# wondmgezahu/RAMP

Hardware: AMD Instinct MI355X
Metric: sampled trajectories/sec (H=48, T=25) (higher is better)
Workload: dtype f32-emulated (2 x fp16 planes per operand, fp32 accumulate)

## Files before the change

### ramp_amd/build.py

```python
from __future__ import annotations

import os
import re
import subprocess
import sys
from concurrent.futures import ThreadPoolExecutor

HERE = os.path.dirname(os.path.abspath(__file__))
CSRC = os.path.join(HERE, "csrc")
LIBDIR = os.path.join(HERE, "lib")
LIB = os.path.join(LIBDIR, "libramp_hip.so")
TOOLS_LIB = os.path.join(LIBDIR, "libramp_hip_tools.so")
SOURCES = ["gemm.hip", "ffx.hip", "ffx16.hip", "tkl.hip", "tkl16.hip", "atk.hip", "atb.hip", "atl.hip", "tkc.hip", "tkw.hip", "rowops.hip", "attention.hip", "sampler.hip", "guide.hip", "guide_replan.hip", "guide_prims.hip", "stitch.hip", "resample.hip", "clearance.hip", "scene.hip", "metrics.hip", "engine.hip", "ops.hip"]
TOOLS_SOURCES = ["bench.hip"]
FLAGS = ["--offload-arch=gfx950", "-O3", "-std=c++17", "-fPIC", "-Wno-unused-result", "-DRAMP_DEFAULT_GEMM_MODE=2"]
EXTRA_FLAGS = {"sampler.hip": ["-ffp-contract=off"], "guide.hip": ["-ffp-contract=off"], "guide_replan.hip": ["-ffp-contract=off"], "guide_prims.hip": ["-ffp-contract=off"], "resample.hip": ["-ffp-contract=off"], "clearance.hip": ["-ffp-contract=off"], "stitch.hip": ["-ffp-contract=off"], "ffx.hip": ["-fno-slp-vectorize"], "ffx16.hip": ["-fno-slp-vectorize"], "tkl.hip": ["-fno-slp-vectorize"], "tkl16.hip": ["-fno-slp-vectorize"], "atk.hip": ["-fno-slp-vectorize", "-mllvm", "-amdgpu-mfma-vgpr-form"], "atb.hip": ["-fno-slp-vectorize"], "atl.hip": ["-fno-slp-vectorize", "-mllvm", "-amdgpu-mfma-vgpr-form"], "tkc.hip": ["-fno-slp-vectorize"], "tkw.hip": ["-fno-slp-vectorize"]}


def _stale(out: str, deps) -> bool:
    if not os.path.exists(out):
        return True
    t = os.path.getmtime(out)
    return any(os.path.getmtime(d) > t for d in deps)


def header_deps():
    import glob
    hs = sorted(glob.glob(os.path.join(CSRC, "*.h")) + glob.glob(os.path.join(CSRC, "*.inc")))
    return hs + [os.path.join(HERE, "..", "include", "ramp_hip.h"), os.path.join(HERE, "..", "include", "ramp_hip_tools.h"), os.path.abspath(__file__)]


_INCLUDE = re.compile(r'^\s*#\s*include\s+"([^"]+)"', re.M)


def source_deps(path: str):
    seen, todo = [], [os.path.normpath(path)]
    while todo:
        f = todo.pop()
        if f in seen or not os.path.exists(f):
            continue
        seen.append(f)
        with open(f, encoding="utf-8") as fh:
            for inc in _INCLUDE.findall(fh.read()):
                todo.append(os.path.normpath(os.path.join(os.path.dirname(f), inc)))
    return seen + [os.path.abspath(__file__)]


def stale_sources(force: bool = False):
    objdir = os.path.join(LIBDIR, "obj")
    jobs = []
    for src in SOURCES + TOOLS_SOURCES:
        sp = os.path.join(CSRC, src)
        op = os.path.join(objdir, src.replace(".hip", ".o"))
        if force or _stale(op, source_deps(sp)):
            jobs.append((sp, op))
    return jobs


def build(force: bool = False, verbose: bool = True) -> str:
    hipcc = os.environ.get("HIPCC", "/opt/rocm/bin/hipcc")
    os.makedirs(LIBDIR, exist_ok=True)
    objdir = os.path.join(LIBDIR, "obj")
    os.makedirs(objdir, exist_ok=True)
    jobs = stale_sources(force)

    def compile_one(job):
        sp, op = job
        cmd = [hipcc] + FLAGS + EXTRA_FLAGS.get(os.path.basename(sp), []) + ["-c", sp, "-o", op]
        r = subprocess.run(cmd, capture_output=True, text=True)
        if r.returncode != 0:
            raise RuntimeError(f"hipcc failed for {sp}:\n{r.stderr[-4000:]}")
        return sp

    if jobs:
        with ThreadPoolExecutor(max_workers=4) as ex:
            for sp in ex.map(compile_one, jobs):
                if verbose:
                    print(f"[ramp_amd.build] compiled {os.path.basename(sp)}", file=sys.stderr)
    objs = [os.path.join(objdir, s.replace(".hip", ".o")) for s in SOURCES]
    tobjs = objs + [os.path.join(objdir, s.replace(".hip", ".o")) for s in TOOLS_SOURCES]
    for lib, oo in ((LIB, objs), (TOOLS_LIB, tobjs)):
        if force or jobs or _stale(lib, oo):
            cmd = [hipcc, "--offload-arch=gfx950", "-shared", "-fPIC", "-o", lib] + oo
            r = subprocess.run(cmd, capture_output=True, text=True)
            if r.returncode != 0:
                raise RuntimeError(f"link failed:\n{r.stderr[-4000:]}")
            if verbose:
                print(f"[ramp_amd.build] linked {lib}", file=sys.stderr)
    return LIB


if __name__ == "__main__":
    build(force="--force" in sys.argv)
```

### ramp_amd/csrc/args_gemm.h

```cpp
#pragma once
#include "core.h"
#include "pack.h"

namespace ramp {

struct GemmArgs {
  const float* A = nullptr;  int lda = 0;
  const float* A2 = nullptr; int lda2 = 0; int K1 = 0;
  const float* W = nullptr;
  const unsigned short* Wx = nullptr; long wx_plane = 0;
  const float* a_absmax_in = nullptr; float* a_absmax_out = nullptr; int* range_flag = nullptr; float w_scale_inv = 1.f;
  int site_id = 0;
  int geglu_group = 64;
  const float* Amul = nullptr; int lda_mul = 0; int a_period = 0;
  int ablate = 0;
  int three_ok = 1;
  int tile_pref = 0;
  int wx_packed = 0;
  const float* bias = nullptr;
  const float* rowbias = nullptr; const int* rowvar = nullptr; int row0 = 0; int rb_stride = 0;
  const float* resid = nullptr;  int ldr = 0;
  const float* resid2 = nullptr; int ldr2 = 0;
  float* C = nullptr;  int ldc = 0;
  float* C2 = nullptr; int ldc2 = 0; int N1 = 0;
  int M = 0, N = 0, K = 0;
  int taps = 1, shift0 = 0, shift_step = 0, L = 1;
  int a_stride = 1, c_rstride = 1, c_roff = 0;
  int epi = 0;
  const float* aux_in = nullptr;
  float* aux_out = nullptr;
  int ld_aux = 0;
};
enum { EPI_LINEAR = 0, EPI_GEGLU_FWD = 1, EPI_GEGLU_BWD = 2 };
int launch_gemm(const GemmArgs& a, hipStream_t s);
int launch_ff_fwd(const GemmArgs& ff1, const GemmArgs& ff2, hipStream_t s);
int init_gemm_attributes();
}
```

### ramp_amd/csrc/gemm.hip

```cpp
#include "args_gemm.h"

#include <algorithm>

namespace ramp {

typedef float f32x16 __attribute__((ext_vector_type(16)));
typedef float f32x4 __attribute__((ext_vector_type(4)));

constexpr int BK = 32;
constexpr int LDS_LD = BK + 4;

__device__ __forceinline__ float gelu_f(float x) { return 0.5f * x * (1.f + erff(x * 0.70710678118654752440f)); }
__device__ __forceinline__ float gelu_grad_f(float x) {
  const float cdf = 0.5f * (1.f + erff(x * 0.70710678118654752440f));
  const float pdf = expf(-0.5f * x * x) * 0.39894228040143267794f;
  return cdf + x * pdf;
}

__device__ __forceinline__ void normal_cdf_pdf(float x, float& cdf, float& pdf) {
  const float ax = fabsf(x);
  const float t = __builtin_amdgcn_rcpf(fmaf(0.2316419f, ax, 1.f));
  pdf = __builtin_amdgcn_exp2f(x * x * -0.72134752044448170368f) * 0.39894228040143267794f;
  float poly = fmaf(1.330274429f, t, -1.821255978f);
  poly = fmaf(poly, t, 1.781477937f);
// ... 926 lines not shown
          }
        }
        parity ^= 1;
      }
      load_w(bw[1], wnext, 0, 1);
      if (a.ablate & 2) {
#pragma unroll
        for (int qq = 0; qq < 4; ++qq) asm volatile("" :: "v"(acc[qq >> 1][qq & 1]));
#pragma unroll
        for (int ni = 0; ni < NI; ++ni) wblk[ni] = wnext[ni];
        __syncthreads();
        continue;
      }
      {
        float* Rw = RAW + wn * (FF_RAW / 4);
#pragma unroll
        for (int mi = 0; mi < MI; ++mi)
#pragma unroll
          for (int ni = 0; ni < NI; ++ni)
#pragma unroll
            for (int reg = 0; reg < 16; ++reg)
              Rw[(mi * 32 + (reg & 3) + 8 * (reg >> 2) + 4 * h) * 68 + ni * 32 + r] = acc[mi][ni][reg];
      }
#pragma unroll
      for (int ni = 0; ni < NI; ++ni) wblk[ni] = wnext[ni];
      __syncthreads();
    }
  } else {
    u32x4 fa[NP][MI], fb[2][NP][NI];
    load_w2(fb[0], 0);
    __syncthreads();
#pragma unroll 1
    for (int it = 0; it < 9; ++it) __syncthreads();
    f32x16 acc[MI][NI];
    for (int cq = 0; cq < Q; ++cq) {
      if ((cq & 7) == 0) {
#pragma unroll
        for (int mi = 0; mi < MI; ++mi)
#pragma unroll
          for (int ni = 0; ni < NI; ++ni)
#pragma unroll
            for (int e = 0; e < 16; ++e) acc[mi][ni][e] = 0.f;
      }
      if (a.ablate & 1) {
#pragma unroll 1
        for (int it = 0; it < 9; ++it) __syncthreads();
        continue;
      }
      const int mtq = mt_begin + (cq >> 3) * mt_step, cidx = cq & 7;
      {
        const float* Rw = RAW + wn * (FF_RAW / 4);
        const int rl0 = lane >> 3, c = (lane & 7) * 4;
        const int nbase = cidx * 256 + wn * 64;
        const int half = a.N >> 1, j0 = cidx * 128 + wn * 32 + c;
        f32x4 ba = {0, 0, 0, 0}, bg = {0, 0, 0, 0};
        if (a.bias) { ba = *reinterpret_cast<const f32x4*>(a.bias + nbase + c); bg = *reinterpret_cast<const f32x4*>(a.bias + nbase + 32 + c); }
        unsigned short* PHw = PH + wn * BUF;
#pragma unroll 1
        for (int it = 0; it < 4; ++it) {
          if (a.ablate & 8) { __syncthreads(); continue; }
#pragma unroll
          for (int p = 0; p < 2; ++p) {
            const int rl = (it * 2 + p) * 8 + rl0, m = mtq * 64 + rl;
            f32x4 av4 = *reinterpret_cast<const f32x4*>(Rw + rl * 68 + c);
            f32x4 gv = *reinterpret_cast<const f32x4*>(Rw + rl * 68 + 32 + c);
            av4 = av4 * oscale1 + ba; gv = gv * oscale1 + bg;
            f32x4 hv, s1, s2;
#pragma unroll
            for (int e = 0; e < 4; ++e) {
              float cdf, pdf;
              normal_cdf_pdf(gv[e], cdf, pdf);
              s1[e] = gv[e] * cdf;
              s2[e] = av4[e] * (cdf + gv[e] * pdf);
              hv[e] = av4[e] * s1[e];
            }
            if (m < a.M) {
              *reinterpret_cast<f32x4*>(a.C + (long)m * a.ldc + j0) = s1;
              *reinterpret_cast<f32x4*>(a.C + (long)m * a.ldc + half + j0) = s2;
            } else {
              hv = f32x4{0, 0, 0, 0};
            }
            amax_h = fmaxf(fmaxf(fabsf(hv[0]), fabsf(hv[1])), amax_h); amax_h = fmaxf(fmaxf(fabsf(hv[2]), fabsf(hv[3])), amax_h);
            scale4(hv, s_h);
            const int c8 = lane & 7;
            const int off = rl * XLD + ((((c8 >> 1) ^ (rl >> 2)) & 3) << 3) + (c8 & 1) * 4;
#pragma unroll
            for (int pp = 0; pp < NP; ++pp) *reinterpret_cast<u32x2*>(PHw + pp * PLANE + off) = peel4<NP>(hv, pp + 1 < NP);
          }
          __syncthreads();
        }
      }
#pragma unroll 1
      for (int it = 0; it < 4; ++it) {
        if (a.ablate & 4) { __syncthreads(); continue; }
        const int kb = cidx * 8 + 2 * it;
        load_w2(fb[1], (kb + 1) & 63);
        read_a(fa, PH + it * BUF, 0);
#pragma unroll
        for (int t3 = 0; t3 < 3; ++t3)
#pragma unroll
          for (int mi = 0; mi < MI; ++mi)
#pragma unroll
            for (int ni = 0; ni < NI; ++ni)
              acc[mi][ni] = mfma_planes<NP>(fa[PA[t3]][mi], fb[0][PB[t3]][ni], acc[mi][ni]);
        load_w2(fb[0], (kb + 2) & 63);
        read_a(fa, PH + it * BUF, 1);
#pragma unroll
        for (int t3 = 0; t3 < 3; ++t3)
#pragma unroll
          for (int mi = 0; mi < MI; ++mi)
#pragma unroll
            for (int ni = 0; ni < NI; ++ni)
              acc[mi][ni] = mfma_planes<NP>(fa[PA[t3]][mi], fb[1][PB[t3]][ni], acc[mi][ni]);
        __syncthreads();
      }
      if ((cq & 7) == 7) {
        epilogue_wave_aux<EPI_LINEAR, false, true, 64, 256, 1>(b, acc, Sw, mtq, 1, lane, 0, wn, r, h, oscale2);
      }
      __syncthreads();
    }
  }

  {
    float mx = G1 ? amax : amax_h;
#pragma unroll
    for (int o = 32; o > 0; o >>= 1) mx = fmaxf(mx, __shfl_xor(mx, o));
    if (lane == 0) {
      const GemmArgs& g = G1 ? a : b;
      const float sc = G1 ? s_a : s_h;
      record_amax(g.a_absmax_out, mx);
      if (g.range_flag && (!(mx * sc < 60000.f) || (mx > 0.f && mx * sc < 0.125f))) atomicMax(g.range_flag, g.site_id + 1);
    }
  }
}

int launch_ff_fwd(const GemmArgs& g1, const GemmArgs& g2, hipStream_t s) {
  auto al16 = [](const void* p) { return (reinterpret_cast<uintptr_t>(p) & 15) == 0; };
  RAMP_REQUIRE(g1.wx_packed == 2 && g2.wx_packed == 2 && g1.Wx && g2.Wx, "fused feed-forward needs the fp16 weight planes");
  RAMP_REQUIRE(g1.K == 256 && g1.N == 2048 && g2.K == 1024 && g2.N == 256 && g1.M == g2.M && g1.M > 0, "fused feed-forward: 256 -> 2 x 1024 -> 256 only");
  RAMP_REQUIRE(g1.geglu_group == 32 && g1.taps == 1 && g2.taps == 1 && !g1.A2 && !g1.Amul && !g2.rowbias && !g2.resid2 && !g2.C2, "fused feed-forward: unsupported operand");
  RAMP_REQUIRE(g1.lda % 4 == 0 && g1.ldc % 4 == 0 && g2.ldc % 4 == 0 && (g2.resid == nullptr || g2.ldr % 4 == 0), "leading dimensions must be multiples of 4 floats");
  RAMP_REQUIRE(al16(g1.A) && al16(g1.Wx) && al16(g2.Wx) && al16(g1.C) && al16(g2.C) && al16(g1.bias) && al16(g2.bias) && al16(g2.resid), "operands must be 16-byte aligned");
  FfFwdArgs f; f.g1 = g1; f.g2 = g2;
  f.g2.N1 = f.g2.N; f.g2.K1 = f.g2.K; f.g1.N1 = f.g1.N; f.g1.K1 = f.g1.K;
  const int n_mtiles = (g1.M + 63) / 64;
  const int nb = std::min(((n_mtiles + 7) / 8) * 8, 256);
  hipLaunchKernelGGL(ff_fwd_kernel, dim3(nb), dim3(512), FF_LDS, s, f, n_mtiles);
  RAMP_HIP_CHECK(hipGetLastError());
  return 0;
}

template <int NP>
__global__ void pack_planes_kernel(const float* __restrict__ W, unsigned short* __restrict__ out, long rows, int K, float scale) {
  const int k8n = K / 8;
  const long total = rows * k8n;
  for (long i = (long)blockIdx.x * 256 + threadIdx.x; i < total; i += (long)gridDim.x * 256) {
    const long row = i / k8n;
    const int k8 = (int)(i - row * k8n);
    f32x4 lo = *reinterpret_cast<const f32x4*>(W + row * K + k8 * 8) * scale;
    f32x4 hi = *reinterpret_cast<const f32x4*>(W + row * K + k8 * 8 + 4) * scale;
    const long blk = (row >> 5) * (K / 16) + (k8 >> 1);
    unsigned short* q = out + blk * (NP * 512) + (((k8 & 1) * 32 + (int)(row & 31)) << 3);
#pragma unroll
    for (int p = 0; p < NP; ++p) {
      const bool sub = p + 1 < NP;
      const u32x2 qa = peel4<NP>(lo, sub), qb = peel4<NP>(hi, sub);
      *reinterpret_cast<u32x4*>(q + p * 512) = u32x4{qa[0], qa[1], qb[0], qb[1]};
    }
  }
}
int launch_pack_x6(const float* W, unsigned short* out, long rows, int K, hipStream_t s) {
  RAMP_REQUIRE(rows > 0 && rows % 32 == 0 && K > 0 && K % 16 == 0, "pack_x6 needs rows % 32 == 0 and K % 16 == 0");
  const long total = rows * (K / 8);
  hipLaunchKernelGGL(pack_planes_kernel<3>, dim3((int)std::min<long>((total + 255) / 256, 8192)), dim3(256), 0, s, W, out, rows, K, 1.f);
  RAMP_HIP_CHECK(hipGetLastError());
  return 0;
}
int launch_pack_h3(const float* W, unsigned short* out, long rows, int K, float scale, hipStream_t s) {
  RAMP_REQUIRE(rows > 0 && rows % 32 == 0 && K > 0 && K % 16 == 0, "pack_h3 needs rows % 32 == 0 and K % 16 == 0");
  const long total = rows * (K / 8);
  hipLaunchKernelGGL(pack_planes_kernel<2>, dim3((int)std::min<long>((total + 255) / 256, 8192)), dim3(256), 0, s, W, out, rows, K, scale);
  RAMP_HIP_CHECK(hipGetLastError());
  return 0;
}

constexpr size_t X6_LDS = std::max<size_t>(6 * (size_t)128 * XLD * 2, (size_t)128 * 132 * 4);
constexpr size_t X6P_LDS3 = 2 * (9216 + 3 * (size_t)128 * XLD * 2);
constexpr size_t X6P_LDS2 = 2 * (9728 + 2 * (size_t)128 * XLD * 2);
constexpr size_t X6P_LDS2R = 2 * (17408 + 2 * (size_t)128 * XLD * 2);
constexpr size_t X6P_LDS2W = 2 * (17408 + 2 * (size_t)64 * XLD * 2);
static_assert(X6P_LDS3 <= X6_LDS, "bf16x6 pipelined layout");

template <int EPI, bool GEN>
static int launch_x6(const GemmArgs& a, hipStream_t s) {
  const bool wide = !GEN && a.wx_packed == 2 && a.N % 256 == 0 && a.tile_pref != 1;
  const int BMt = wide ? 64 : 128, BNt = wide ? 256 : 128;
  const int tiles_m = (a.M + BMt - 1) / BMt, tiles_n = (a.N + BNt - 1) / BNt;
  const int n_tiles = tiles_m * tiles_n;
  const bool three_auto = a.three_ok != 0;
  const bool plain = three_auto && EPI == EPI_LINEAR && wide && !a.Amul && !a.resid && !a.rowbias;
  const bool three = a.wx_packed == 2 && (!a.Amul || wide) &&
                     (EPI == EPI_GEGLU_FWD || a.tile_pref == 3 ||
                      (a.tile_pref == 0 && ((plain && n_tiles >= 3072) || (three_auto && wide && a.Amul && n_tiles > 512 && n_tiles <= 768))));
  const int slots = three ? 768 : 512;
  const int rounds = (n_tiles + slots - 1) / slots;
  const int nb = std::min((((n_tiles + rounds - 1) / rounds + 7) / 8) * 8, slots);
#define X6P_LAUNCH(...) hipLaunchKernelGGL((gemm_x6p_kernel<__VA_ARGS__>), dim3(nb), dim3(256), X6P_LDS3, s, a, tiles_n, n_tiles)
  const bool rec = a.a_absmax_out != nullptr;
  if (a.ablate && a.wx_packed == 2) {
    if constexpr (!GEN && EPI == EPI_LINEAR) {
      const size_t lds = wide ? X6P_LDS2W : X6P_LDS2R;
#define ABL_CASE(V) case V: if (wide) hipLaunchKernelGGL((gemm_x6p_abl_kernel<V, true>), dim3(nb), dim3(256), lds, s, a, tiles_n, n_tiles); \
                            else hipLaunchKernelGGL((gemm_x6p_abl_kernel<V, false>), dim3(nb), dim3(256), lds, s, a, tiles_n, n_tiles); break;
      switch (a.ablate) { ABL_CASE(1) ABL_CASE(2) ABL_CASE(3) ABL_CASE(4) ABL_CASE(7) ABL_CASE(8) ABL_CASE(15) ABL_CASE(16) ABL_CASE(32) ABL_CASE(64) ABL_CASE(128) ABL_CASE(136) ABL_CASE(129) ABL_CASE(130) ABL_CASE(131) ABL_CASE(160) ABL_CASE(192) ABL_CASE(144) ABL_CASE(288) ABL_CASE(416) default: RAMP_REQUIRE(false, "ablation variant not built"); }
#undef ABL_CASE
    }
  } else if (wide) {
    if constexpr (!GEN) {
      if (a.Amul) {
        RAMP_REQUIRE(EPI == EPI_LINEAR && a.a_period > 0 && a.a_period % 32 == 0 && a.K == 2 * a.a_period && a.lda_mul % 4 == 0, "bad A-multiplier operand (K = 2 x period)");
        if constexpr (EPI == EPI_LINEAR) {
          if (three) hipLaunchKernelGGL((gemm_x6p3_kernel<EPI_LINEAR, false, true, 2, true, true, true>), dim3(nb), dim3(256), X6P_LDS2W, s, a, tiles_n, n_tiles);
          else hipLaunchKernelGGL((gemm_x6p_kernel<EPI_LINEAR, false, true, 2, true, true>), dim3(nb), dim3(256), X6P_LDS2W, s, a, tiles_n, n_tiles);
        }
      } else if (three && EPI == EPI_LINEAR && !a.resid && !a.rowbias) hipLaunchKernelGGL((gemm_x6p3_kernel<EPI, false, false, 2, true, true, true>), dim3(nb), dim3(256), X6P_LDS2W, s, a, tiles_n, n_tiles);
      else if (three) hipLaunchKernelGGL((gemm_x6p3_kernel<EPI, false, false, 2, true, true>), dim3(nb), dim3(256), X6P_LDS2W, s, a, tiles_n, n_tiles);
      else hipLaunchKernelGGL((gemm_x6p_kernel<EPI, false, false, 2, true, true>), dim3(nb), dim3(256), X6P_LDS2W, s, a, tiles_n, n_tiles);
    }
  } else if (a.wx_packed && a.Amul) {
    RAMP_REQUIRE(EPI == EPI_LINEAR && !GEN && a.a_period > 0 && a.a_period % 32 == 0 && a.K == 2 * a.a_period && a.lda_mul % 4 == 0, "bad A-multiplier operand (K = 2 x period)");
    if (a.wx_packed == 2) hipLaunchKernelGGL((gemm_x6p_kernel<EPI_LINEAR, false, true, 2, true>), dim3(nb), dim3(256), X6P_LDS2R, s, a, tiles_n, n_tiles);
    else if (rec) X6P_LAUNCH(EPI_LINEAR, false, true, 3, true);
    else X6P_LAUNCH(EPI_LINEAR, false, true, 3, false);
  } else if (three) hipLaunchKernelGGL((gemm_x6p3_kernel<EPI, GEN>), dim3(nb), dim3(256), X6P_LDS2, s, a, tiles_n, n_tiles);
  else if (a.wx_packed == 2) hipLaunchKernelGGL((gemm_x6p_kernel<EPI, GEN, false, 2, true>), dim3(nb), dim3(256), X6P_LDS2R, s, a, tiles_n, n_tiles);
  else if (a.wx_packed && rec) X6P_LAUNCH(EPI, GEN, false, 3, true);
  else if (a.wx_packed) X6P_LAUNCH(EPI, GEN, false, 3, false);
  else hipLaunchKernelGGL((gemm_x6_kernel<EPI, GEN>), dim3(nb), dim3(256), X6_LDS, s, a, tiles_n, n_tiles);
  RAMP_HIP_CHECK(hipGetLastError());
  return 0;
}
template <int EPI, bool GEN>
static int set_attr_x6() {
  RAMP_HIP_CHECK(hipFuncSetAttribute(reinterpret_cast<const void*>(&gemm_x6_kernel<EPI, GEN>),
                                     hipFuncAttributeMaxDynamicSharedMemorySize, (int)X6_LDS));
#define X6P_ATTR(...) RAMP_HIP_CHECK(hipFuncSetAttribute(reinterpret_cast<const void*>(&gemm_x6p_kernel<__VA_ARGS__>), \
                                                         hipFuncAttributeMaxDynamicSharedMemorySize, (int)X6P_LDS3))
  X6P_ATTR(EPI, GEN, false, 3, false);
  X6P_ATTR(EPI, GEN, false, 3, true);
  RAMP_HIP_CHECK(hipFuncSetAttribute(reinterpret_cast<const void*>(&gemm_x6p3_kernel<EPI, GEN>),
                                     hipFuncAttributeMaxDynamicSharedMemorySize, (int)X6P_LDS2));
  RAMP_HIP_CHECK(hipFuncSetAttribute(reinterpret_cast<const void*>(&gemm_x6p_kernel<EPI, GEN, false, 2, true>),
                                     hipFuncAttributeMaxDynamicSharedMemorySize, (int)X6P_LDS2R));
  if constexpr (!GEN) {
    RAMP_HIP_CHECK(hipFuncSetAttribute(reinterpret_cast<const void*>(&gemm_x6p_kernel<EPI, false, false, 2, true, true>),
                                       hipFuncAttributeMaxDynamicSharedMemorySize, (int)X6P_LDS2W));
    RAMP_HIP_CHECK(hipFuncSetAttribute(reinterpret_cast<const void*>(&gemm_x6p3_kernel<EPI, false, false, 2, true, true>),
                                       hipFuncAttributeMaxDynamicSharedMemorySize, (int)X6P_LDS2W));
  }
  return 0;
}
template <int WM, int WN, int MI, int NI> struct Cfg {
  static constexpr int BM = WM * MI * 32, BN = WN * NI * 32;
  static constexpr size_t lds = 2 * (size_t)(BM + BN) * LDS_LD * sizeof(float);
};

template <int WM, int WN, int MI, int NI, int EPI, bool GEN>
static int launch_cfg(const GemmArgs& a, int blocks_per_cu, hipStream_t s) {
  using C = Cfg<WM, WN, MI, NI>;
  const int tiles_m = (a.M + C::BM - 1) / C::BM, tiles_n = (a.N + C::BN - 1) / C::BN;
  const int n_tiles = tiles_m * tiles_n;
  const int slots = 256 * blocks_per_cu;
  const int rounds = (n_tiles + slots - 1) / slots;
  const int nb = std::min((((n_tiles + rounds - 1) / rounds + 7) / 8) * 8, slots);
  hipLaunchKernelGGL((gemm_kernel<WM, WN, MI, NI, EPI, GEN>), dim3(nb), dim3(WM * WN * 64), C::lds, s, a, tiles_n, n_tiles);
  RAMP_HIP_CHECK(hipGetLastError());
  return 0;
}

template <int WM, int WN, int MI, int NI, int EPI, bool GEN>
static int set_attr() {
  RAMP_HIP_CHECK(hipFuncSetAttribute(reinterpret_cast<const void*>(&gemm_kernel<WM, WN, MI, NI, EPI, GEN>),
                                     hipFuncAttributeMaxDynamicSharedMemorySize, (int)Cfg<WM, WN, MI, NI>::lds));
  return 0;
}
int init_gemm_attributes() {
  RAMP_HIP_CHECK(hipFuncSetAttribute(reinterpret_cast<const void*>(&ff_fwd_kernel), hipFuncAttributeMaxDynamicSharedMemorySize, (int)FF_LDS));
  if (int e = set_attr<2, 2, 2, 2, EPI_LINEAR, false>()) return e;
  if (int e = set_attr<2, 2, 2, 2, EPI_LINEAR, true>()) return e;
  if (int e = set_attr<2, 2, 2, 2, EPI_GEGLU_FWD, false>()) return e;
  if (int e = set_attr<2, 2, 2, 2, EPI_GEGLU_BWD, false>()) return e;
  if (int e = set_attr<2, 2, 2, 1, EPI_LINEAR, true>()) return e;
  if (int e = set_attr<4, 1, 1, 1, EPI_LINEAR, true>()) return e;
  X6P_ATTR(EPI_LINEAR, false, true, 3, false);
  X6P_ATTR(EPI_LINEAR, false, true, 3, true);
  RAMP_HIP_CHECK(hipFuncSetAttribute(reinterpret_cast<const void*>(&gemm_x6p_kernel<EPI_LINEAR, false, true, 2, true>),
                                     hipFuncAttributeMaxDynamicSharedMemorySize, (int)X6P_LDS2R));
  RAMP_HIP_CHECK(hipFuncSetAttribute(reinterpret_cast<const void*>(&gemm_x6p_kernel<EPI_LINEAR, false, true, 2, true, true>),
                                     hipFuncAttributeMaxDynamicSharedMemorySize, (int)X6P_LDS2W));
#define ABL_ATTR(V) RAMP_HIP_CHECK(hipFuncSetAttribute(reinterpret_cast<const void*>(&gemm_x6p_abl_kernel<V, true>), hipFuncAttributeMaxDynamicSharedMemorySize, (int)X6P_LDS2W)); \
                    RAMP_HIP_CHECK(hipFuncSetAttribute(reinterpret_cast<const void*>(&gemm_x6p_abl_kernel<V, false>), hipFuncAttributeMaxDynamicSharedMemorySize, (int)X6P_LDS2R));
  ABL_ATTR(1) ABL_ATTR(2) ABL_ATTR(3) ABL_ATTR(4) ABL_ATTR(7) ABL_ATTR(8) ABL_ATTR(15) ABL_ATTR(16) ABL_ATTR(32) ABL_ATTR(64)
#undef ABL_ATTR
  if (int e = set_attr_x6<EPI_LINEAR, false>()) return e;
  if (int e = set_attr_x6<EPI_LINEAR, true>()) return e;
  if (int e = set_attr_x6<EPI_GEGLU_FWD, false>()) return e;
  return set_attr_x6<EPI_GEGLU_BWD, false>();
}

__global__ __launch_bounds__(256) void gemm_narrow_kernel(GemmArgs a) {
  const int n4 = a.N >> 2;
  const long idx = (long)blockIdx.x * 256 + threadIdx.x;
  if (idx >= (long)a.M * n4) return;
  const int m = (int)(idx / n4), n = (int)(idx - (long)m * n4) * 4;
  const int seg = m / a.L, l = m - seg * a.L;
  const int Lin = a.L * a.a_stride;
  f32x4 acc = {0, 0, 0, 0};
  for (int tap = 0; tap < a.taps; ++tap) {
    const int ls = l * a.a_stride + a.shift0 + tap * a.shift_step;
    if (ls < 0 || ls >= Lin) continue;
    const long src = (long)seg * Lin + ls;
    const float* w = a.W + ((long)tap * a.N + n) * a.K;
    for (int k = 0; k < a.K; ++k) {
      const float x = k < a.K1 ? a.A[src * a.lda + k] : a.A2[src * a.lda2 + (k - a.K1)];
#pragma unroll
      for (int j = 0; j < 4; ++j) acc[j] += x * w[(long)j * a.K + k];
    }
  }
  const long orow = (long)m * a.c_rstride + a.c_roff;
  if (a.bias) acc += *reinterpret_cast<const f32x4*>(a.bias + n);
  if (a.rowbias) acc += *reinterpret_cast<const f32x4*>(a.rowbias + (long)a.rowvar[a.row0 + m / a.L] * a.rb_stride + n);
  if (a.resid) acc += *reinterpret_cast<const f32x4*>(a.resid + orow * a.ldr + n);
  if (a.resid2) acc += *reinterpret_cast<const f32x4*>(a.resid2 + orow * a.ldr2 + n);
  if (n < a.N1) *reinterpret_cast<f32x4*>(a.C + orow * a.ldc + n) = acc;
  else *reinterpret_cast<f32x4*>(a.C2 + orow * a.ldc2 + (n - a.N1)) = acc;
}

int launch_gemm(const GemmArgs& a_in, hipStream_t s) {
  GemmArgs a = a_in;
  if (a.A2 == nullptr) a.K1 = a.K;
  if (a.C2 == nullptr) a.N1 = a.N;
  if (a.rb_stride == 0) a.rb_stride = a.N;
  auto al16 = [](const void* p) { return (reinterpret_cast<uintptr_t>(p) & 15) == 0; };
  RAMP_REQUIRE(a.M > 0 && a.N > 0 && a.K > 0 && a.taps >= 1 && a.L >= 1, "bad GEMM dims");
  if (a.K % BK != 0) {
    RAMP_REQUIRE(a.K % 16 == 0 && a.N % 4 == 0 && a.N1 % 4 == 0 && a.epi == EPI_LINEAR && !a.Amul && a.a_stride >= 1 && a.c_rstride >= 1 &&
                 (a.A2 == nullptr || a.K1 > 0) && (a.C2 == nullptr || a.N1 > 0),
                 "narrow GEMM (K % 32 != 0): K a multiple of 16, N and N1 multiples of 4, linear epilogue only");
    RAMP_REQUIRE(al16(a.C) && al16(a.C2) && al16(a.resid) && al16(a.resid2) && al16(a.bias) && al16(a.rowbias) &&
                 a.ldc % 4 == 0 && a.ldc2 % 4 == 0 && a.ldr % 4 == 0 && a.ldr2 % 4 == 0 && a.rb_stride % 4 == 0 &&
                 (a.rowbias == nullptr || a.rowvar != nullptr), "narrow GEMM: outputs and epilogue operands must be 16-byte aligned");
    const long n_out = (long)a.M * (a.N / 4);
    hipLaunchKernelGGL(gemm_narrow_kernel, dim3((unsigned)((n_out + 255) / 256)), dim3(256), 0, s, a);
    RAMP_HIP_CHECK(hipGetLastError());
    return 0;
  }
  RAMP_REQUIRE(a.K % BK == 0 && a.lda % 4 == 0 && a.N % 4 == 0 && a.N1 % 4 == 0,
               "K must be a multiple of 32, N, N1 and lda multiples of 4 floats");
  RAMP_REQUIRE(a.A2 == nullptr || (a.lda2 % 4 == 0 && a.K1 % BK == 0), "split-K source must start on a K tile");
  RAMP_REQUIRE(al16(a.A) && al16(a.W) && al16(a.A2) && al16(a.C) && al16(a.C2) && al16(a.resid) && al16(a.resid2) &&
               al16(a.bias) && al16(a.rowbias) && al16(a.aux_in) && al16(a.aux_out), "GEMM operands must be 16-byte aligned");
  RAMP_REQUIRE(a.ldc % 4 == 0 && a.ldc2 % 4 == 0 && a.ldr % 4 == 0 && a.ldr2 % 4 == 0 && a.ld_aux % 4 == 0 &&
               a.rb_stride % 4 == 0, "leading dimensions must be multiples of 4 floats");
  RAMP_REQUIRE(a.rowbias == nullptr || a.rowvar != nullptr, "rowbias needs rowvar");
  RAMP_REQUIRE(a.a_stride >= 1 && a.c_rstride >= 1, "bad strides");
  const bool gen = a.taps > 1 || a.a_stride != 1 || a.c_rstride != 1 || a.c_roff != 0 || a.A2 || a.C2 || a.resid2 ||
                   a.shift0 != 0;
  const bool x6 = a.Wx != nullptr && (a.N >= 128 || (a.wx_packed && a.N >= 64));
  RAMP_REQUIRE(a.Amul == nullptr || (x6 && a.wx_packed && !gen && a.epi == EPI_LINEAR && al16(a.Amul)),
               "the A-multiplier operand needs the pipelined bf16x6 kernel");
  RAMP_REQUIRE(!x6 || (al16(a.Wx) && a.K % 8 == 0 && (a.wx_packed ? a.N % 32 == 0 : a.wx_plane > 0)), "bad bf16x6 weight planes");
  if (a.epi == EPI_GEGLU_FWD) {
    RAMP_REQUIRE(!gen && a.N % 256 == 0 && a.aux_out && !a.resid && !a.rowbias,
                 "GEGLU-forward epilogue needs a plain linear with N % 256 == 0 and aux_out");
    RAMP_REQUIRE((x6 && a.wx_packed != 0) == (a.geglu_group == 32), "GEGLU weight tiling: [32 a | 32 g] for the pipelined kernels, [64 a | 64 g] otherwise");
    if (x6) return launch_x6<EPI_GEGLU_FWD, false>(a, s);
    return launch_cfg<2, 2, 2, 2, EPI_GEGLU_FWD, false>(a, 2, s);
  }
  if (a.epi == EPI_GEGLU_BWD) {
    RAMP_REQUIRE(!gen && a.N >= 128 && a.aux_in && !a.resid && !a.rowbias && !a.bias,
                 "GEGLU-backward epilogue needs a plain linear with aux_in");
    if (x6) return launch_x6<EPI_GEGLU_BWD, false>(a, s);
    return launch_cfg<2, 2, 2, 2, EPI_GEGLU_BWD, false>(a, 2, s);
  }
  if (x6) return gen ? launch_x6<EPI_LINEAR, true>(a, s) : launch_x6<EPI_LINEAR, false>(a, s);
  if (a.N >= 128) {
    if (!gen) return launch_cfg<2, 2, 2, 2, EPI_LINEAR, false>(a, 2, s);
    return launch_cfg<2, 2, 2, 2, EPI_LINEAR, true>(a, 2, s);
  }
  if (a.N >= 64) return launch_cfg<2, 2, 2, 1, EPI_LINEAR, true>(a, 2, s);
  return launch_cfg<4, 1, 1, 1, EPI_LINEAR, true>(a, 3, s);
}

}
```

Before: 4097.

## Add persistent weight-resident GEMM kernel for large-M narrow linear layers

Adds a persistent kernel that loads the entire packed weight matrix into LDS once per block, then loops over 32-token row groups. Each group's activations are prefetched into registers, and the split-precision MFMA products are computed with a fused bias/scale/residual epilogue. It is routed for plain linear GEMMs with K,N in {64,128,256} and M at or above a threshold. The aim is to avoid re-reading weights per tile and to cut tile-launch overhead for tall, skinny GEMMs. In exchange it uses one wave per EU with large LDS, and an env switch can disable it.

Result: no change. 4109, median of 6 (+0.3%).

```diff
diff --git a/ramp_amd/build.py b/ramp_amd/build.py
--- a/ramp_amd/build.py
+++ b/ramp_amd/build.py
@@ -11,10 +11,10 @@
 LIBDIR = os.path.join(HERE, "lib")
 LIB = os.path.join(LIBDIR, "libramp_hip.so")
 TOOLS_LIB = os.path.join(LIBDIR, "libramp_hip_tools.so")
-SOURCES = ["gemm.hip", "ffx.hip", "ffx16.hip", "tkl.hip", "tkl16.hip", "atk.hip", "atb.hip", "atl.hip", "tkc.hip", "tkw.hip", "rowops.hip", "attention.hip", "sampler.hip", "guide.hip", "guide_replan.hip", "guide_prims.hip", "stitch.hip", "resample.hip", "clearance.hip", "scene.hip", "metrics.hip", "engine.hip", "ops.hip"]
+SOURCES = ["gemm.hip", "gemm_edge.hip", "ffx.hip", "ffx16.hip", "tkl.hip", "tkl16.hip", "atk.hip", "atb.hip", "atl.hip", "tkc.hip", "tkw.hip", "rowops.hip", "attention.hip", "sampler.hip", "guide.hip", "guide_replan.hip", "guide_prims.hip", "stitch.hip", "resample.hip", "clearance.hip", "scene.hip", "metrics.hip", "engine.hip", "ops.hip"]
 TOOLS_SOURCES = ["bench.hip"]
 FLAGS = ["--offload-arch=gfx950", "-O3", "-std=c++17", "-fPIC", "-Wno-unused-result", "-DRAMP_DEFAULT_GEMM_MODE=2"]
-EXTRA_FLAGS = {"sampler.hip": ["-ffp-contract=off"], "guide.hip": ["-ffp-contract=off"], "guide_replan.hip": ["-ffp-contract=off"], "guide_prims.hip": ["-ffp-contract=off"], "resample.hip": ["-ffp-contract=off"], "clearance.hip": ["-ffp-contract=off"], "stitch.hip": ["-ffp-contract=off"], "ffx.hip": ["-fno-slp-vectorize"], "ffx16.hip": ["-fno-slp-vectorize"], "tkl.hip": ["-fno-slp-vectorize"], "tkl16.hip": ["-fno-slp-vectorize"], "atk.hip": ["-fno-slp-vectorize", "-mllvm", "-amdgpu-mfma-vgpr-form"], "atb.hip": ["-fno-slp-vectorize"], "atl.hip": ["-fno-slp-vectorize", "-mllvm", "-amdgpu-mfma-vgpr-form"], "tkc.hip": ["-fno-slp-vectorize"], "tkw.hip": ["-fno-slp-vectorize"]}
+EXTRA_FLAGS = {"sampler.hip": ["-ffp-contract=off"], "guide.hip": ["-ffp-contract=off"], "guide_replan.hip": ["-ffp-contract=off"], "guide_prims.hip": ["-ffp-contract=off"], "resample.hip": ["-ffp-contract=off"], "clearance.hip": ["-ffp-contract=off"], "stitch.hip": ["-ffp-contract=off"], "ffx.hip": ["-fno-slp-vectorize"], "ffx16.hip": ["-fno-slp-vectorize"], "tkl.hip": ["-fno-slp-vectorize"], "tkl16.hip": ["-fno-slp-vectorize"], "gemm_edge.hip": ["-fno-slp-vectorize"], "atk.hip": ["-fno-slp-vectorize", "-mllvm", "-amdgpu-mfma-vgpr-form"], "atb.hip": ["-fno-slp-vectorize"], "atl.hip": ["-fno-slp-vectorize", "-mllvm", "-amdgpu-mfma-vgpr-form"], "tkc.hip": ["-fno-slp-vectorize"], "tkw.hip": ["-fno-slp-vectorize"]}
 
 
 def _stale(out: str, deps) -> bool:
diff --git a/ramp_amd/csrc/args_gemm.h b/ramp_amd/csrc/args_gemm.h
--- a/ramp_amd/csrc/args_gemm.h
+++ b/ramp_amd/csrc/args_gemm.h
@@ -35,4 +35,7 @@
 int launch_gemm(const GemmArgs& a, hipStream_t s);
 int launch_ff_fwd(const GemmArgs& ff1, const GemmArgs& ff2, hipStream_t s);
 int init_gemm_attributes();
+bool gemm_edge_serves(const GemmArgs& a);
+int launch_gemm_edge(const GemmArgs& a, hipStream_t s);
+int init_gemm_edge_attributes();
 }
diff --git a/ramp_amd/csrc/gemm.hip b/ramp_amd/csrc/gemm.hip
--- a/ramp_amd/csrc/gemm.hip
+++ b/ramp_amd/csrc/gemm.hip
@@ -1252,6 +1252,7 @@
                     RAMP_HIP_CHECK(hipFuncSetAttribute(reinterpret_cast<const void*>(&gemm_x6p_abl_kernel<V, false>), hipFuncAttributeMaxDynamicSharedMemorySize, (int)X6P_LDS2R));
   ABL_ATTR(1) ABL_ATTR(2) ABL_ATTR(3) ABL_ATTR(4) ABL_ATTR(7) ABL_ATTR(8) ABL_ATTR(15) ABL_ATTR(16) ABL_ATTR(32) ABL_ATTR(64)
 #undef ABL_ATTR
+  if (int e = init_gemm_edge_attributes()) return e;
   if (int e = set_attr_x6<EPI_LINEAR, false>()) return e;
   if (int e = set_attr_x6<EPI_LINEAR, true>()) return e;
   if (int e = set_attr_x6<EPI_GEGLU_FWD, false>()) return e;
@@ -1333,6 +1334,7 @@
     if (x6) return launch_x6<EPI_GEGLU_BWD, false>(a, s);
     return launch_cfg<2, 2, 2, 2, EPI_GEGLU_BWD, false>(a, 2, s);
   }
+  if (x6 && !gen && gemm_edge_serves(a)) return launch_gemm_edge(a, s);
   if (x6) return gen ? launch_x6<EPI_LINEAR, true>(a, s) : launch_x6<EPI_LINEAR, false>(a, s);
   if (a.N >= 128) {
     if (!gen) return launch_cfg<2, 2, 2, 2, EPI_LINEAR, false>(a, 2, s);
diff --git a/ramp_amd/csrc/gemm_edge.hip b/ramp_amd/csrc/gemm_edge.hip
--- /dev/null
+++ b/ramp_amd/csrc/gemm_edge.hip
@@ -0,0 +1,187 @@
+#include "args_gemm.h"
+#include "tokmma.h"
+
+#include <algorithm>
+#include <cstdlib>
+#include <type_traits>
+
+namespace ramp {
+
+namespace {
+constexpr int GE_TROW = 36;
+constexpr int GE_SCR = 32 * GE_TROW * 4;
+constexpr size_t ge_lds(int K, int N) { return (size_t)K * N * 4 + 4 * GE_SCR + (size_t)N * 4; }
+static_assert(ge_lds(256, 128) <= 160 * 1024 && ge_lds(128, 256) <= 160 * 1024, "LDS budget");
+}
+
+namespace {
+template <int I, int E, class Fn>
+__device__ __forceinline__ void static_for(Fn&& f) {
+  if constexpr (I < E) { f(std::integral_constant<int, I>{}); static_for<I + 1, E>(f); }
+}
+}
+
+template <int K, int N, bool RES>
+__global__ __launch_bounds__(256) __attribute__((amdgpu_waves_per_eu(1, 1)))
+void gemm_edge_kernel(GemmArgs a, int n_groups) {
+  constexpr int NKS = K / 16, NB = N / 32;
+  constexpr int NLD = K / 8;
+  constexpr int W_BYTES = K * N * 4;
+  extern __shared__ __attribute__((aligned(16))) char smem[];
+  const int tid = threadIdx.x, lane = tid & 63;
+  const int wave = __builtin_amdgcn_readfirstlane(tid >> 6);
+  const int t = lane & 31, h = lane >> 5;
+
+  const float s_a = scale_of(a.a_absmax_in);
+  const float os = a.w_scale_inv / s_a;
+  float amax = 0.f;
+
+  f32x4 xn[NLD];
+  auto x_row = [&](int g) __attribute__((always_inline)) {
+    long tok = (long)g * 32 + t;
+    tok = tok < a.M ? tok : a.M - 1;
+    return a.A + tok * a.lda + 8 * h;
+  };
+  const int stride = (int)gridDim.x * 4;
+  int g = (int)blockIdx.x * 4 + wave;
+  {
+    const float* xr = x_row(g);
+#pragma unroll
+    for (int u = 0; u < NLD; ++u) xn[u] = *reinterpret_cast<const f32x4*>(xr + 16 * (u >> 1) + 4 * (u & 1));
+  }
+  {
+    const char* wsrc = reinterpret_cast<const char*>(a.Wx) + lane * 16;
+    const unsigned wdst = (unsigned)(uintptr_t)smem;
+#pragma unroll
+    for (int i = 0; i < W_BYTES / 4096; ++i) {
+      const int piece = 4 * i + wave;
+      asm volatile("s_mov_b32 m0, %1\n\ts_nop 0\n\tglobal_load_lds_dwordx4 %0, off" :: "v"(wsrc + piece * 1024), "s"(wdst + piece * 1024) : "memory", "m0");
+    }
+    float* bsw = reinterpret_cast<float*>(smem + W_BYTES + 4 * GE_SCR);
+    for (int i = tid; i < N; i += 256) bsw[i] = a.bias ? a.bias[i] : 0.f;
+  }
+  asm volatile("s_waitcnt vmcnt(0)" ::: "memory");
+  __syncthreads();
+
+  const char* wrd = smem + lane * 16;
+  const int l8 = lane >> 3, c4 = 4 * (lane & 7);
+  float* tw = reinterpret_cast<float*>(smem + W_BYTES + wave * GE_SCR);
+  float* tw_w = tw + t * GE_TROW + 4 * h;
+  const float* tw_r = tw + l8 * GE_TROW + c4;
+  const float* bs = reinterpret_cast<const float*>(smem + W_BYTES + 4 * GE_SCR) + c4;
+
+  for (; g < n_groups; g += stride) {
+    const float* xr_next = x_row(g + stride < n_groups ? g + stride : g);
+    u32x4 XB[NKS][2];
+#pragma unroll
+    for (int ks = 0; ks < NKS; ++ks) {
+      amax_pin(amax, xn[2 * ks][0], xn[2 * ks][1]); amax_pin(amax, xn[2 * ks][2], xn[2 * ks][3]);
+      amax_pin(amax, xn[2 * ks + 1][0], xn[2 * ks + 1][1]); amax_pin(amax, xn[2 * ks + 1][2], xn[2 * ks + 1][3]);
+      split8(xn[2 * ks] * s_a, xn[2 * ks + 1] * s_a, XB[ks][0], XB[ks][1]);
+      xn[2 * ks] = *reinterpret_cast<const f32x4*>(xr_next + 16 * ks);
+      xn[2 * ks + 1] = *reinterpret_cast<const f32x4*>(xr_next + 16 * ks + 4);
+      __builtin_amdgcn_sched_barrier(0);
+    }
+    auto row_of = [&](int j) __attribute__((always_inline)) {
+      const long r_ = (long)g * 32 + 8 * j + l8;
+      return r_ < a.M ? r_ : (long)a.M - 1;
+    };
+
+    f32x16 acc[2];
+    f32x4 rz[2][4];
+    auto epi = [&](const f32x16& P, const f32x4 (&r)[4], int fb) __attribute__((always_inline)) {
+#pragma unroll
+      for (int q = 0; q < 4; ++q) *reinterpret_cast<f32x4*>(tw_w + 8 * q) = quad(P, q);
+      const f32x4 bq = *reinterpret_cast<const f32x4*>(bs + 32 * fb);
+#pragma unroll
+      for (int j = 0; j < 4; ++j) {
+        f32x4 v = *reinterpret_cast<const f32x4*>(tw_r + 8 * j * GE_TROW) * os + bq;
+        if (RES) v += r[j];
+        *reinterpret_cast<f32x4*>(a.C + row_of(j) * a.ldc + 32 * fb + c4) = v;
+      }
+    };
+    u32x4 F[4][2];
+    auto frag = [&](const char* base, int i) __attribute__((always_inline)) {
+      F[i & 3][0] = *reinterpret_cast<const u32x4*>(base + i * 2048);
+      F[i & 3][1] = *reinterpret_cast<const u32x4*>(base + i * 2048 + 1024);
+    };
+    frag(wrd, 0); frag(wrd, 1); frag(wrd, 2);
+#pragma unroll 1
+    for (int pr = 0; pr < NB / 2; ++pr) {
+      const char* base = wrd + pr * (2 * NKS * 2048);
+      static_for<0, 2 * NKS>([&](auto si) __attribute__((always_inline)) {
+        constexpr int i = decltype(si)::value, half = i / NKS, ks = i % NKS;
+        const int fb = 2 * pr + half;
+        f32x16& ac = acc[half];
+        if (ks == 0) {
+          if (RES) {
+#pragma unroll
+            for (int j = 0; j < 4; ++j) rz[half][j] = *reinterpret_cast<const f32x4*>(a.resid + row_of(j) * a.ldr + 32 * fb + c4);
+          }
+#pragma unroll
+          for (int e = 0; e < 16; ++e) ac[e] = 0.f;
+        }
+        if (i + 3 < 2 * NKS || pr + 1 < NB / 2) frag(base, i + 3);
+        ac = mfma16(F[i & 3][1], XB[ks][0], ac);
+        ac = mfma16(F[i & 3][0], XB[ks][1], ac);
+        ac = mfma16(F[i & 3][0], XB[ks][0], ac);
+        if (ks == 1 && half == 1) epi(acc[0], rz[0], fb - 1);
+        if (ks == 1 && half == 0 && pr > 0) epi(acc[1], rz[1], fb - 1);
+        __builtin_amdgcn_sched_barrier(0);
+      });
+    }
+    epi(acc[1], rz[1], NB - 1);
+  }
+
+#pragma unroll
+  for (int o = 32; o > 0; o >>= 1) amax = fmaxf(amax, __shfl_xor(amax, o));
+  record_amax_block_guarded(a.a_absmax_out, amax, reinterpret_cast<float*>(smem), a.range_flag, s_a, a.site_id);
+}
+
+static int edge_switch() {
+  const char* e = getenv("RAMP_EDGE");
+  return e ? atoi(e) : 1;
+}
+
+constexpr int GEMM_EDGE_MIN_M = 32768;
+
+bool gemm_edge_serves(const GemmArgs& a) {
+  const int sw = edge_switch();
+  if (sw == 0) return false;
+  auto dim_ok = [](int d) { return d == 64 || d == 128 || d == 256; };
+  const bool plain = a.taps == 1 && a.a_stride == 1 && a.c_rstride == 1 && a.c_roff == 0 && a.shift0 == 0 && !a.A2 && !a.C2 && !a.resid2;
+  const bool built = a.wx_packed == 2 && a.Wx && plain && a.epi == EPI_LINEAR && !a.Amul && !a.rowbias && !a.ablate && a.tile_pref == 0 &&
+                     dim_ok(a.K) && dim_ok(a.N) && !(a.K == 256 && a.N == 256) && a.lda % 4 == 0 && a.ldc % 4 == 0 && (!a.resid || a.ldr % 4 == 0) &&
+                     !ranges_overlap(a.C, ((size_t)(a.M - 1) * a.ldc + a.N) * 4, a.A, ((size_t)(a.M - 1) * a.lda + a.K) * 4) &&
+                     !ranges_overlap(a.C, ((size_t)(a.M - 1) * a.ldc + a.N) * 4, a.resid, ((size_t)(a.M - 1) * a.ldr + a.N) * 4);
+  const bool faster = a.M >= GEMM_EDGE_MIN_M && !(a.K == 256 && a.N == 128);
+  return built && (faster || sw == 2);
+}
+
+#define GE_SHAPES(X) X(64, 64) X(64, 128) X(64, 256) X(128, 64) X(128, 128) X(128, 256) X(256, 64) X(256, 128)
+
+int launch_gemm_edge(const GemmArgs& a, hipStream_t s) {
+  RAMP_REQUIRE(a.M > 0 && a.A && a.C && a.Wx, "gemm_edge: bad operand");
+  const int n_groups = (a.M + 31) / 32;
+  const int nb = std::min((n_groups + 3) / 4, device_cu_count());
+#define GE_GO(KK, NN)                                                                                                                  \
+  if (a.K == KK && a.N == NN) {                                                                                                        \
+    if (a.resid) hipLaunchKernelGGL((gemm_edge_kernel<KK, NN, true>), dim3(nb), dim3(256), ge_lds(KK, NN), s, a, n_groups);           \
+    else hipLaunchKernelGGL((gemm_edge_kernel<KK, NN, false>), dim3(nb), dim3(256), ge_lds(KK, NN), s, a, n_groups);                  \
+  } else
+  GE_SHAPES(GE_GO) RAMP_REQUIRE(false, "gemm_edge: shape not built");
+#undef GE_GO
+  RAMP_HIP_CHECK(hipGetLastError());
+  return 0;
+}
+
+int init_gemm_edge_attributes() {
+#define GE_ATTR(KK, NN)                                                                                                                \
+  RAMP_HIP_CHECK(hipFuncSetAttribute(reinterpret_cast<const void*>(&gemm_edge_kernel<KK, NN, true>), hipFuncAttributeMaxDynamicSharedMemorySize, (int)ge_lds(KK, NN))); \
+  RAMP_HIP_CHECK(hipFuncSetAttribute(reinterpret_cast<const void*>(&gemm_edge_kernel<KK, NN, false>), hipFuncAttributeMaxDynamicSharedMemorySize, (int)ge_lds(KK, NN)));
+  GE_SHAPES(GE_ATTR)
+#undef GE_ATTR
+  return 0;
+}
+
+}
```
